# jw007123/hp-Adaptive-Signed-Distance-Field-Octree

Hardware: AMD Instinct MI355X
Metric: Query() Mpts/sec at targetError=1e-5 (union3 field, 10M SplitMix64 pts per GPU, HBM-resident); Create() ms reported as create_ms (higher is better)
Workload: dtype f64

## Files before the change

### hp-adaptive-signed-distance-field-octree_amd/csrc/field_eval.hpp

```cpp
#pragma once
#include <hip/hip_runtime.h>

#include "device_types.hpp"

namespace hpsdf {

template <bool LEFT>
__device__ __forceinline__ double sum3(double a, double b, double c) {
    if constexpr (LEFT) return (a + b) + c;
    else return a + (b + c);
}
template <bool LEFT>
__device__ __forceinline__ double prod3(double a, double b, double c) {
    if constexpr (LEFT) return (a * b) * c;
    else return a * (b * c);
}
__device__ __forceinline__ double sqrtExact(double x) {
    const uint32_t hi = (uint32_t)__double2hiint(x);
    const bool plain = hi - 0x10000000u < 0x7FF00000u - 0x10000000u;
    if (__builtin_amdgcn_ballot_w64(!plain) != 0ull) return sqrt(x);
    const double y = __builtin_amdgcn_rsq(x);
    double g = x * y, h = y * 0.5;
    const double r = __builtin_fma(-h, g, 0.5);
    g = __builtin_fma(g, r, g);
    h = __builtin_fma(h, r, h);
    double d = __builtin_fma(-g, g, x);
    g = __builtin_fma(d, h, g);
    d = __builtin_fma(-g, g, x);
    return __builtin_fma(d, h, g);
}

template <bool LEFT>
__device__ __forceinline__ double norm3(double x, double y, double z) { return sqrtExact(sum3<LEFT>(x * x, y * y, z * z)); }

template <bool LEFT>
__device__ __forceinline__ double primEval(const hpsdf_prim& pr, double x, double y, double z) {
    const double* p = pr.p;
    switch (pr.kind) {
        case HPSDF_PRIM_SPHERE:
            return norm3<LEFT>(x - p[0], y - p[1], z - p[2]) - p[3];
        case HPSDF_PRIM_BOX: {
            const double qx = fabs(x - p[0]) - p[3];
            const double qy = fabs(y - p[1]) - p[4];
            const double qz = fabs(z - p[2]) - p[5];
            const double outside = norm3<LEFT>(fmax(qx, 0.0), fmax(qy, 0.0), fmax(qz, 0.0));
            const double inside = fmin(fmax(qx, fmax(qy, qz)), 0.0);
            return outside + inside;
        }
        case HPSDF_PRIM_TORUS_Y: {
            const double dx = x - p[0], dy = y - p[1], dz = z - p[2];
            const double l = sqrtExact(dx * dx + dz * dz) - p[3];
            return sqrtExact(l * l + dy * dy) - p[4];
        }
        case HPSDF_PRIM_PLANE:
            return (p[0] * x + (p[1] * y + p[2] * z)) + p[3];
        default:
            return 0.0;
    }
}

template <bool LEFT>
__device__ __forceinline__ double analyticEval(const FieldDev& f, double x, double y, double z) {
    double acc = primEval<LEFT>(f.prims[0], x, y, z);
    for (int i = 1; i < f.nPrims; ++i) {
        const double d = primEval<LEFT>(f.prims[i], x, y, z);
        switch (f.prims[i].op) {
            case HPSDF_OP_UNION: acc = fmin(acc, d); break;
            case HPSDF_OP_INTERSECT: acc = fmax(acc, d); break;
            default: acc = fmax(acc, -d); break;
        }
    }
    return acc;
}

}
```

### hp-adaptive-signed-distance-field-octree_amd/csrc/fit_analytic.hip

```cpp
#include "fit_kernels.hpp"

namespace hpsdf {

HPSDF_FIT_KIND_UNIT(, kFieldAnalytic)

}
```

### hp-adaptive-signed-distance-field-octree_amd/csrc/fit_kernels.hpp

```cpp
#pragma once
#include <hip/hip_runtime.h>

#include <cstdint>

#include "device_types.hpp"
#include "field_glue.hpp"
#include "launch.hpp"

namespace hpsdf {


constexpr int kFitPiece = 8;
#ifndef HPSDF_FIT_MIN_WAVES
#define HPSDF_FIT_MIN_WAVES 4
#endif

__device__ __forceinline__ double fitRowAny(double acc, double a1, const double* __restrict__ tk, double n2,
                                            const double* __restrict__ F, int nq) {
    int k = 0;
    for (; k + 4 <= nq; k += 4) {
        const double f0 = F[k], f1 = F[k + 1], f2 = F[k + 2], f3 = F[k + 3];
        const double t0 = tk[k], t1 = tk[k + 1], t2 = tk[k + 2], t3 = tk[k + 3];
        acc = acc + (a1 * t0 * n2) * f0;
        acc = acc + (a1 * t1 * n2) * f1;
        acc = acc + (a1 * t2 * n2) * f2;
        acc = acc + (a1 * t3 * n2) * f3;
    }
    for (; k < nq; ++k) acc = acc + (a1 * tk[k] * n2) * F[k];
    return acc;
}

template <int KIND, bool CSG, int DEG, int R, bool LEFT>
__device__ __forceinline__ void fitBlockBody(const FitBlock blk, const FitTask* __restrict__ tasks, double* __restrict__ arena,
                                             double* __restrict__ errs, double* __restrict__ mirror,
                                             const DeviceTables* __restrict__ T, const FieldDev& field, const RootMap& rm, double* lds) {
    static_assert(R == 1 || DEG > 0, "cell blocking needs a compile-time degree");
    __shared__ double sNl[13 * 11];
    __shared__ double sRec[26];
    __shared__ int32_t sMeshStack[kFitThreads / 64][kMeshStack];
    __shared__ unsigned char sPosI[KIND == kFieldMesh ? 64 : 4], sPosJK[KIND == kFieldMesh ? 64 : 4];
    const int tid = threadIdx.x;
    const int deg = DEG > 0 ? DEG : (int)blk.degree;
    const int nq = 4 * deg + 1, nq2 = nq * nq, G = blk.nTasks;
    const int rowStart = blk.rowStart, rowEnd = blk.rowEnd, nrows = rowEnd - rowStart;
    const int gl = nq * (nq - 1) / 2;
    const int planes = blk.planesPerChunk;
    const int depth = blk.depth;
    const bool split = blk.split != 0;

    double* sT = lds;
    double* sR = sT + (deg + 1) * nq;
    double* sW = sR + nq;
    double* sC = sW + nq;
    double* sF = sC + 8 * G;

    stageQueryTables(T, sNl, sRec);
    for (int q = tid; q < nq; q += kFitThreads) {
        const double x = T->roots[gl + q];
        sR[q] = x;
        sW[q] = T->weights[gl + q];
        double m2 = 0.0, m1 = 1.0;
        sT[q] = 1.0;
        for (int i = 1; i <= deg; ++i) {
            const double l = T->rec[i][0] * x * m1 - T->rec[i][1] * m2;
            m2 = m1, m1 = l;
            sT[i * nq + q] = l;
        }
    }
    for (int g = tid; g < G; g += kFitThreads) {
        const FitTask& tk = tasks[blk.firstTask + g];
        double sc[3];
        for (int a = 0; a < 3; ++a) {
            sc[a] = (double)(tk.bmax[a] - tk.bmin[a]) * 0.5;
            sC[8 * g + 3 + a] = (double)((tk.bmin[a] + tk.bmax[a]) / 2.0f);
            sC[8 * g + a] = sc[a];
        }
        sC[8 * g + 6] = prod3<LEFT>(sc[0], sc[1], sc[2]);
        sC[8 * g + 7] = __longlong_as_double((long long)tk.sampleOff);
    }
    __syncthreads();

    const bool wide = DEG == 0 && nrows > kFitThreads;
    const int slot = wide ? 0 : tid / nrows;
    const int g2 = slot * R;
    const int r0 = rowStart + (wide ? tid : tid % nrows);
    const int r1 = r0 + kFitThreads;
    const bool act0 = wide ? (r0 < rowEnd) : (tid < ((G + R - 1) / R) * nrows);
    const bool act1 = wide && r1 < rowEnd;
    int i0a = 0, i1a = 0, i2a = 0, i0b = 0, i1b = 0, i2b = 0;
    double n0a = 0, n1a = 0, n2a = 0, n0b = 0, n1b = 0, n2b = 0;
    if (act0) {
        i0a = T->bidx[r0][0], i1a = T->bidx[r0][1], i2a = T->bidx[r0][2];
        n0a = sNl[i0a * 11 + depth], n1a = sNl[i1a * 11 + depth], n2a = sNl[i2a * 11 + depth];
    }
    if (act1) {
        i0b = T->bidx[r1][0], i1b = T->bidx[r1][1], i2b = T->bidx[r1][2];
        n0b = sNl[i0b * 11 + depth], n1b = sNl[i1b * 11 + depth], n2b = sNl[i2b * 11 + depth];
    }
    constexpr int NQF = DEG > 0 ? 4 * DEG + 1 : 1;
    double tkReg[NQF];
    if (DEG > 0) {
#pragma unroll
        for (int k = 0; k < NQF; ++k) tkReg[k] = sT[i2a * nq + k];
    }
    uint32_t meshHint = 0xFFFFFFFFu;
    double acc[R];
#pragma unroll
    for (int r = 0; r < R; ++r) acc[r] = 0.0;
    double acc1 = 0.0;

    const int cellStride = planes * nq2;
    for (int iBase = 0; iBase < nq; iBase += planes) {
        const int np = min(planes, nq - iBase);
        if constexpr (KIND == kFieldMesh) {
            if (tid < nq) {
                int rank = 0;
                for (int b = 0; b < nq; ++b) rank += sR[b] < sR[tid] ? 1 : 0;
                sPosJK[rank] = (unsigned char)tid;
            }
            if (tid >= 64 && tid < 64 + np) {
                const int a = tid - 64;
                int rank = 0;
                for (int b = 0; b < np; ++b) rank += sR[iBase + b] < sR[iBase + a] ? 1 : 0;
                sPosI[rank] = (unsigned char)a;
            }
            __syncthreads();
        }
        if constexpr (KIND != kFieldMesh) {
            const int cols = G * nq2;
            for (int c0 = 0; c0 < cols; c0 += kFitThreads) {
                const int cc = c0 + tid;
                const bool activeS = cc < cols;
                const int ccl = activeS ? cc : cols - 1;
                const int g = ccl / nq2, jk = ccl - g * nq2, j = jk / nq, k = jk - j * nq;
                const double* c = sC + 8 * g;
                const double uy = sR[j] * c[1] + c[4], uz = sR[k] * c[2] + c[5];
                const double wy = uy * rm.bounds[1] + rm.centre[1];
                const double wz = uz * rm.bounds[2] + rm.centre[2];
                const double wj = sW[j], wk = sW[k], c6 = c[6];
                const uint64_t sbase = (uint64_t)__double_as_longlong(c[7]) + (uint64_t)(j * nq + k);
                for (int il = 0; il < np; ++il) {
                    const int i = iBase + il;
                    const double ux = sR[i] * c[0] + c[3];
                    const double wx = ux * rm.bounds[0] + rm.centre[0];
                    const uint64_t sidx = sbase + (uint64_t)(i * nq2);
                    const double fv = activeS ? fieldEvalWorld<KIND, CSG, LEFT>(field, wx, wy, wz, sidx, sNl, sRec, meshHint) : 0.0;
                    if (activeS) {
                        sF[g * cellStride + il * nq2 + jk] = c6 * prod3<LEFT>(sW[i], wj, wk) * fv;
                        if (split) const_cast<double*>(field.samples)[sidx] = fv;
                    }
                }
            }
        } else {
            const int chunkSamples = np * nq2, total = G * chunkSamples;
            const float invChunk = 1.0f / (float)chunkSamples;
            for (int s0 = 0; s0 < total; s0 += kFitThreads) {
                const int s = s0 + tid;
                const bool activeS = s < total;
                const int sc = activeS ? s : total - 1;
                int g = (int)(((float)sc + 0.5f) * invChunk);
                int rem = sc - g * chunkSamples;
                if (rem < 0) {
                    --g;
                    rem += chunkSamples;
                } else if (rem >= chunkSamples) {
                    ++g;
                    rem -= chunkSamples;
                }
                if constexpr (KIND == kFieldMesh) rem = meshSampleOrder(rem, np, nq, sPosI, sPosJK);
                const double* c = sC + 8 * g;
                const int il = rem / nq2, jk = rem - il * nq2, j = jk / nq, k = jk - j * nq, i = iBase + il;
                const double ux = sR[i] * c[0] + c[3], uy = sR[j] * c[1] + c[4], uz = sR[k] * c[2] + c[5];
                const double wx = ux * rm.bounds[0] + rm.centre[0];
                const double wy = uy * rm.bounds[1] + rm.centre[1];
                const double wz = uz * rm.bounds[2] + rm.centre[2];
                const uint64_t sidx = (uint64_t)__double_as_longlong(c[7]) + (uint64_t)((i * nq + j) * nq + k);
                double fv;
                if constexpr (KIND == kFieldMesh) {
                    const double mv = (double)meshSignedDistanceWave(field.mesh, V3{(float)wx, (float)wy, (float)wz}, activeS, meshHint,
                                                                     sMeshStack[tid >> 6]);
                    fv = activeS ? applyCsg<CSG>(field, mv, wx, wy, wz, sNl, sRec) : 0.0;
                } else {
                    fv = activeS ? fieldEvalWorld<KIND, CSG, LEFT>(field, wx, wy, wz, sidx, sNl, sRec, meshHint) : 0.0;
                }
                if (activeS) {
                    sF[g * cellStride + rem] = c[6] * prod3<LEFT>(sW[i], sW[j], sW[k]) * fv;
                    if constexpr (KIND != kFieldMesh)
                        if (split) const_cast<double*>(field.samples)[sidx] = fv;
                }
            }
        }
        __syncthreads();
        if (act0) {
            const double* tj = sT + i1a * nq;
            const double* tk = sT + i2a * nq;
            for (int il = 0; il < np; ++il) {
                const double* F = sF + g2 * cellStride + il * nq2;
                const double a0 = sT[i0a * nq + iBase + il] * n0a;
#ifdef HPSDF_FIT_ROW_UNROLL
#pragma unroll HPSDF_FIT_ROW_UNROLL
#endif
                for (int j = 0; j < nq; ++j) {
                    const double a1 = a0 * tj[j] * n1a;
                    if constexpr (DEG > 0 && DEG <= 5) {
                        double lp[NQF];
#pragma unroll
                        for (int k = 0; k < NQF; ++k) lp[k] = a1 * tkReg[k] * n2a;
#pragma unroll
                        for (int r = 0; r < R; ++r) {
                            const double* Fr = F + r * cellStride + j * nq;
                            double f[NQF];
#pragma unroll
                            for (int k = 0; k < NQF; ++k) f[k] = Fr[k];
#pragma unroll
                            for (int k = 0; k < NQF; ++k) acc[r] = acc[r] + lp[k] * f[k];
                        }
                    } else if constexpr (DEG > 5) {
                        const double* Fr = F + j * nq;
#pragma unroll
                        for (int k0 = 0; k0 < NQF; k0 += kFitPiece) {
                            double lp[kFitPiece], f[kFitPiece];
#pragma unroll
                            for (int k = 0; k < kFitPiece; ++k)
                                if (k0 + k < NQF) f[k] = Fr[k0 + k];
#pragma unroll
                            for (int k = 0; k < kFitPiece; ++k)
                                if (k0 + k < NQF) lp[k] = a1 * tkReg[k0 + k] * n2a;
#pragma unroll
                            for (int k = 0; k < kFitPiece; ++k)
                                if (k0 + k < NQF) acc[0] = acc[0] + lp[k] * f[k];
                        }
                    } else {
                        acc[0] = fitRowAny(acc[0], a1, tk, n2a, F + j * nq, nq);
                    }
                }
            }
        }
        if (act1) {
            const double* tj = sT + i1b * nq;
            const double* tk = sT + i2b * nq;
            for (int il = 0; il < np; ++il) {
                const double* F = sF + il * nq2;
                const double a0 = sT[i0b * nq + iBase + il] * n0b;
                for (int j = 0; j < nq; ++j) {
                    const double a1 = a0 * tj[j] * n1b;
                    acc1 = fitRowAny(acc1, a1, tk, n2b, F + j * nq, nq);
                }
            }
        }
        __syncthreads();
    }

    const bool weighted = blk.weighted != 0;
    const int stashStride = weighted ? rowEnd : nrows, stashBase = weighted ? 0 : rowStart;
    const int outBase = split ? 0 : stashBase;
    if (act0) {
#pragma unroll
        for (int r = 0; r < R; ++r)
            if (g2 + r < G) {
                const uint64_t at = tasks[blk.firstTask + g2 + r].outOff + (r0 - outBase);
                arena[at] = acc[r];
                if (mirror != nullptr) mirror[at] = acc[r];
                sF[(g2 + r) * stashStride + (r0 - stashBase)] = acc[r];
            }
    }
    if (act1) {
        arena[tasks[blk.firstTask].outOff + (r1 - outBase)] = acc1;
        sF[r1 - stashBase] = acc1;
    }
    if (weighted && rowStart > 0) {
        for (int s = tid; s < G * rowStart; s += kFitThreads) {
            const int g = s / rowStart, r = s - g * rowStart;
            const FitTask& tk = tasks[blk.firstTask + g];
            const double v = arena[tk.copyOff + r];
            arena[tk.outOff + r] = v;
            sF[g * stashStride + r] = v;
        }
    }
    __syncthreads();
    for (int g = tid; g < G; g += kFitThreads) {
        const int first = deg > 0 ? (int)T->count[deg - 1] : 0;
        double e = 0.0;
        for (int r = first > rowStart ? first : rowStart; r < rowEnd; ++r)
            if (T->bidx[r][3] == deg) {
                const double c = sF[g * stashStride + (r - stashBase)];
                e = e + c * c;
            }
        errs[tasks[blk.firstTask + g].errSlot] = e;
    }
}

template <int KIND, bool CSG, bool LEFT>
__global__ __launch_bounds__(kFitThreads, HPSDF_FIT_MIN_WAVES) void fit_multi_kernel(const FitBlock* __restrict__ blocks,
                                                                const FitTask* __restrict__ tasks, double* __restrict__ arena,
                                                                double* __restrict__ errs, const DeviceTables* __restrict__ T,
                                                                FieldDev field, RootMap rm, const uint32_t* __restrict__ count,
                                                                uint32_t countValue) {
    extern __shared__ double lds[];
    const uint32_t n = count ? *count : countValue;
    if (blockIdx.x >= n) return;
    const FitBlock blk = blocks[n - 1u - blockIdx.x];
    switch (blk.degree) {
        case 2: fitBlockBody<KIND, CSG, 2, 1, LEFT>(blk, tasks, arena, errs, nullptr, T, field, rm, lds); break;
        case 3: fitBlockBody<KIND, CSG, 3, 1, LEFT>(blk, tasks, arena, errs, nullptr, T, field, rm, lds); break;
        case 4: fitBlockBody<KIND, CSG, 4, 1, LEFT>(blk, tasks, arena, errs, nullptr, T, field, rm, lds); break;
        case 5: fitBlockBody<KIND, CSG, 5, 1, LEFT>(blk, tasks, arena, errs, nullptr, T, field, rm, lds); break;
        case 6: fitBlockBody<KIND, CSG, 6, 1, LEFT>(blk, tasks, arena, errs, nullptr, T, field, rm, lds); break;
        case 7: fitBlockBody<KIND, CSG, 7, 1, LEFT>(blk, tasks, arena, errs, nullptr, T, field, rm, lds); break;
        case 8: fitBlockBody<KIND, CSG, 8, 1, LEFT>(blk, tasks, arena, errs, nullptr, T, field, rm, lds); break;
        default: fitBlockBody<KIND, CSG, 0, 1, LEFT>(blk, tasks, arena, errs, nullptr, T, field, rm, lds); break;
    }
}

template <int KIND, bool CSG, int DEG, int R, bool LEFT>
__global__ __launch_bounds__(kFitThreads, HPSDF_FIT_MIN_WAVES) void fit_kernel(const FitBlock* __restrict__ blocks,
                                                          const FitTask* __restrict__ tasks, double* __restrict__ arena,
                                                          double* __restrict__ errs, double* __restrict__ mirror,
                                                          const DeviceTables* __restrict__ T, FieldDev field, RootMap rm,
                                                          const uint32_t* __restrict__ range) {
    extern __shared__ double lds[];
    uint32_t b = blockIdx.x;
    if (range != nullptr) {
        if (b >= range[1]) return;
        b += range[0];
    }
    fitBlockBody<KIND, CSG, DEG, R, LEFT>(blocks[b], tasks, arena, errs, mirror, T, field, rm, lds);
}

template <int KIND, bool CSG, bool LEFT>
__global__ __launch_bounds__(256) void field_kernel(FieldDev f, const DeviceTables* __restrict__ T,
                                                    const double* __restrict__ xyz, size_t n, double* __restrict__ out) {
    __shared__ double sNl[13 * 11];
    __shared__ double sRec[26];
    stageQueryTables(T, sNl, sRec);
    __syncthreads();
    const size_t stride = (size_t)gridDim.x * blockDim.x;
    uint32_t hint = 0xFFFFFFFFu;
    for (size_t i = (size_t)blockIdx.x * blockDim.x + threadIdx.x; i < n; i += stride)
        out[i] = fieldEvalWorld<KIND, CSG, LEFT>(f, xyz[3 * i], xyz[3 * i + 1], xyz[3 * i + 2], i, sNl, sRec, hint);
}

template <int KIND, bool CSG, bool LEFT>
// ... 83 lines not shown
```

### hp-adaptive-signed-distance-field-octree_amd/csrc/frontier.hip

```cpp
#include <hip/hip_runtime.h>

#include <algorithm>
#include <atomic>
#include <cfloat>
#include <cmath>
#include <cstddef>
#include <chrono>
#include <cstdio>
#include <cstdlib>
#include <cstring>
#include <memory>
#include <vector>

#include "block.hpp"
#include "builder.hpp"
#include "frontier.hpp"
#include "launch.hpp"
#include "runtime.hpp"

namespace hpsdf {

namespace {

constexpr uint32_t kFrJobs = 4096;
// ... 98 lines not shown
    int32_t fastFit;
    int32_t splitFit;
    uint64_t sampleCap;
    uint32_t buildStamp;
    uint32_t stamps;
    double target;
    int32_t weighted;
    int32_t replica;
    double* means;
    const double* weights;
    uint32_t* hostFlag;
};

__host__ __device__ inline uint32_t frCoef(int p) { return p == 6 ? 83u : (uint32_t)((p + 1) * (p + 2) * (p + 3) / 6); }
__host__ __device__ inline int frClass(int degree, bool incr, int depth) { return (2 * degree + (incr ? 1 : 0)) * kFrDepths + depth; }
__host__ __device__ inline size_t frLds(int degree, int g, int planes) {
    const size_t nq = 4 * (size_t)degree + 1;
    return ((size_t)(degree + 1) * nq + 2 * nq + 8 * (size_t)g + (size_t)g * planes * nq * nq) * sizeof(double);
}
constexpr size_t kFrFitLdsCap = 45 * 1024;
__host__ __device__ inline bool frSplit(int splitFit, int degree, bool incr) { return splitFit > 0 && !incr && degree >= splitFit && degree <= 11; }
__host__ __device__ inline void frShape(int degree, bool incr, uint32_t count, int* cells, int* planes, bool fast = false, bool weighted = false,
                                        int split = 0) {
    if (fast && degree >= 4 && degree <= 11) {
        *cells = kMfmaCells, *planes = 1;
        return;
    }
    if (frSplit(split, degree, incr)) incr = true;
    const int nrows = incr ? (int)(frCoef(degree) - frCoef(degree - 1)) : (int)frCoef(degree);
    int gmax = nrows > kFitBlockThreads ? 1 : kFitBlockThreads / nrows;
    while (gmax > 1 && frLds(degree, gmax, 1) > (weighted ? kFitMaxLdsBytes : kFrFitLdsCap)) --gmax;
    uint32_t spread = (count + 511u) / 512u;
    int cap = gmax;
    if (degree == 2) {
        if (count <= 4096u) spread = (count + 1023u) / 1024u;
        cap = gmax < 16 ? gmax : 16;
    }
    int g = (int)(spread < 1u ? 1u : spread);
    g = g < cap ? g : cap;
    const int nq = 4 * degree + 1;
    int pl = nq;
    while (pl > 1 && frLds(degree, g, pl) > kFitChunkLdsBytes) --pl;
    if (weighted) {
        const int need = (int)frCoef(degree) + 100;
        const int minPlanes = (need + nq * nq - 1) / (nq * nq);
        const int want = nq < minPlanes ? nq : minPlanes;
        pl = pl > want ? pl : want;
        while (g > 1 && frLds(degree, g, pl) > kFitMaxLdsBytes) --g;
    }
    *cells = g;
    *planes = pl;
}

__device__ __forceinline__ size_t frErrSlot(const FrDev& d, const FrHdr* h, uint32_t j) {
    if (d.world == 1) return (size_t)j * 9;
    const uint32_t o = d.jobOwner[j];
    return (size_t)o * d.errStride + (size_t)(j - h->sliceFirst[o]) * 9;
}
__device__ __forceinline__ double* frStatusSlot(const FrDev& d, int r) { return d.errs + (size_t)r * d.errStride + (d.errStride - 1u); }
__device__ __forceinline__ void frPeerCheck(const FrDev& d, uint32_t* sPeer) {
    if (d.world > 1 && threadIdx.x < (uint32_t)d.world &&
        (unsigned long long)__double_as_longlong(*(volatile double*)frStatusSlot(d, (int)threadIdx.x)) == ~0ull)
        atomicMax(sPeer, threadIdx.x + 1u);
}
__device__ __forceinline__ uint64_t frJobCost(int degree, int depth, bool coarse) {
    auto cube = [](uint64_t n) { return n * n * n; };
    if (coarse) return frCoef(2) * cube(9);
    uint64_t c = 0;
    if (depth < kMaxDepth) c += 8ull * frCoef(degree) * cube(4 * (uint64_t)degree + 1);
    if (degree < kMaxDegree - 1) c += (uint64_t)(frCoef(degree + 1) - frCoef(degree)) * cube(4 * (uint64_t)degree + 5);
    return c ? c : 1;
}

__device__ __forceinline__ uint32_t frDigit(int level, uint64_t bits, uint32_t idx) {
    switch (level) {
        case 0: return (uint32_t)(bits >> 52) & 2047u;
        case 1: return (uint32_t)(bits >> 41) & 2047u;
        case 2: return (uint32_t)(bits >> 30) & 2047u;
        case 3: return (uint32_t)(bits >> 19) & 2047u;
        case 4: return (uint32_t)(bits >> 8) & 2047u;
        case 5: return (uint32_t)bits & 255u;
        case 6: return (~idx >> 21) & 2047u;
        case 7: return (~idx >> 10) & 2047u;
        default: return ~idx & 1023u;
    }
}

__device__ void frThreshold(const uint32_t* hist, uint32_t need, uint32_t* , int* outT, uint32_t* outAbove) {
    if (threadIdx.x < 64) {
        const int lane = (int)threadIdx.x;
        uint32_t own = 0;
        for (int k = 0; k < 32; ++k) own += hist[lane * 32 + k];
        uint32_t suf = own;
        for (int off = 1; off < 64; off <<= 1) {
            const uint32_t v = __shfl_down(suf, off, 64);
            if (lane + off < 64) suf += v;
        }
        const uint32_t aboveLane = suf - own;
        const bool crossing = aboveLane < need && need <= suf;
        const unsigned long long m = __ballot(crossing);
        if (m == 0ull) {
            if (lane == 0) *outT = -1, *outAbove = suf;
        } else if (crossing) {
            uint32_t cum = aboveLane;
            int bb = lane * 32 + 31;
            for (; bb > lane * 32 && cum + hist[bb] < need; --bb) cum += hist[bb];
// ... 1435 lines not shown
        d.segFirst[i] = 2;
    }
    if (blockIdx.x != 0) return;
    if (threadIdx.x == 0 && d.world > 1) *frStatusSlot(d, d.rank) = 0.0;
    uint32_t* hw = reinterpret_cast<uint32_t*>(d.hdr);
    for (uint32_t w = threadIdx.x; w < sizeof(FrHdr) / 4; w += 256u) hw[w] = 0;
    __syncthreads();
    if (threadIdx.x == 0) {
        FrHdr* h = d.hdr;
        h->nNodes = t.nNodes;
        h->nJobs = t.nLeaves;
        h->nLeaves = t.nLeaves;
        h->t1 = -1;
        h->total = 4096.0 * HPSDF_INITIAL_NODE_ERR;
        h->maxDegree = 2;
        h->nTasks = t.nTasks, h->nBlocks = t.nBlocks;
        h->degTasks[2][0] = 0, h->degTasks[2][1] = t.nTasks;
        h->degBlocks[2][0] = 0, h->degBlocks[2][1] = t.nBlocks;
        h->arenaUsed = t.arenaRows;
        h->sampleUsed = t.samples;
        h->fits = t.nTasks, h->samples = t.samples;
        h->nCoeffs = (uint64_t)t.nLeaves * frCoef(2);
        for (int r = 0; r < 9; ++r) h->sliceFirst[r] = t.sliceFirst[r];
    }
    if (d.world > 1)
        for (uint32_t j = threadIdx.x; j < t.nLeaves; j += 256u) {
            uint32_t o = 0;
            for (int r = 1; r < d.world; ++r) o += t.sliceFirst[r] <= j ? 1u : 0u;
            d.jobOwner[j] = (uint8_t)o;
        }
}

}

struct FrontierWorkspace {
    int device = -1;
    bool inUse = false;
    FrDev d{};
    FrHdr* hostHdr = nullptr;
    uint32_t nodeCap = 0;
    uint64_t arenaCap = 0, sampleCap = 0;
    double* arena = nullptr;
    double* samples = nullptr;
    FrTemplate tmpl{};
    hpsdf_node* tmplNodes = nullptr;
    uint32_t* tmplParent = nullptr;
    uint32_t* tmplSub = nullptr;
    uint32_t* tmplLeaves = nullptr;
    double* tmplErr = nullptr;
    uint64_t* tmplJobP = nullptr;
    FitTask* tmplTasks = nullptr;
    FitBlock* tmplBlocks = nullptr;
    size_t tmplLds = 0;
    bool clean = false;
    bool lastWentOn = false;
    int cleanRank = -1, cleanWorld = -1;
    uint32_t buildStamp = 0;
    std::vector<hpsdf_node> hostNodesAfterRound0;
    char* pinned = nullptr;
    double* pinnedDev = nullptr;
    size_t pinnedCap = 0;
    double* hostMeans = nullptr;
    double* hostWeights = nullptr;
    uint32_t* hostFlag = nullptr;
    uint32_t flagStamp = 0;
    hipError_t ensureWeighting() {
        if (hostMeans) return hipSuccess;
        const size_t n = 8 * ((size_t)kFrJobs * HPSDF_JOB_HEADER_DOUBLES + kFrStatusPad);
        hipError_t e = hipHostMalloc((void**)&hostMeans, n * sizeof(double), hipHostMallocCoherent | hipHostMallocMapped);
        if (e == hipSuccess) e = hipHostMalloc((void**)&hostWeights, n * sizeof(double), hipHostMallocCoherent | hipHostMallocMapped);
        if (e == hipSuccess) e = hipHostMalloc((void**)&hostFlag, 64, hipHostMallocCoherent | hipHostMallocMapped);
        if (e == hipSuccess) e = hipHostGetDevicePointer((void**)&d.means, hostMeans, 0);
        if (e == hipSuccess) e = hipHostGetDevicePointer((void**)&d.weights, hostWeights, 0);
        if (e == hipSuccess) e = hipHostGetDevicePointer((void**)&d.hostFlag, hostFlag, 0);
        if (e == hipSuccess) {
            std::memset(hostMeans, 0, n * sizeof(double));
            for (size_t i = 0; i < n; ++i) hostWeights[i] = 1.0;
            hostFlag[0] = hostFlag[1] = 0;
        }
        return e;
    }
    static constexpr int kSide = 3;
    hipStream_t side[kSide] = {nullptr, nullptr, nullptr};
    hipEvent_t forkEv = nullptr, joinEv[kSide] = {nullptr, nullptr, nullptr};

    template <typename T>
    static hipError_t grow(T** p, size_t oldCount, size_t newCount, hipStream_t s, bool keep) {
        T* np = nullptr;
        hipError_t e = hipMalloc((void**)&np, newCount * sizeof(T));
        if (e != hipSuccess) return e;
        if (*p) {
            if (keep && oldCount) e = hipMemcpyAsync(np, *p, oldCount * sizeof(T), hipMemcpyDeviceToDevice, s);
            if (e == hipSuccess) e = hipStreamSynchronize(s);
            (void)hipFree(*p);
        }
        *p = np;
        return e;
    }
    static constexpr uint64_t kBytesPerNode = sizeof(hpsdf_node) + sizeof(uint64_t)  + 2 * sizeof(uint32_t)  +
                                              (uint64_t)kFrSegs * sizeof(uint64_t)  + sizeof(uint64_t)  + 2 * sizeof(uint32_t) ;
    hipError_t ensureNodes(uint32_t need, hipStream_t s) {
        if (need <= nodeCap) return hipSuccess;
        uint32_t nc = nodeCap ? nodeCap : 65536u;
        while (nc < need) nc *= 2;
        hipError_t e = grow(&d.nodes, nodeCap, nc, s, true);
        if (e == hipSuccess) e = grow(&d.qErr, nodeCap, nc, s, true);
// ... 66 lines not shown
        size_t nc = pinnedCap ? pinnedCap : (1u << 20);
        while (nc < need) nc *= 2;
        if (pinned) (void)hipHostFree(pinned);
        pinned = nullptr, pinnedDev = nullptr, pinnedCap = 0;
        hipError_t e = hipHostMalloc((void**)&pinned, nc, hipHostMallocCoherent | hipHostMallocMapped);
        if (e == hipSuccess) e = hipHostGetDevicePointer((void**)&pinnedDev, pinned, 0);
        if (e == hipSuccess) pinnedCap = nc;
        return e;
    }
    template <typename T>
    static hipError_t upload(T** dst, const std::vector<T>& v) {
        hipError_t e = hipMalloc((void**)dst, std::max<size_t>(1, v.size()) * sizeof(T));
        if (e == hipSuccess && !v.empty()) e = hipMemcpy(*dst, v.data(), v.size() * sizeof(T), hipMemcpyHostToDevice);
        return e;
    }
    hipError_t init(int dev, hipStream_t s) {
        device = dev;
        hipError_t e = hipMalloc((void**)&d.hdr, sizeof(FrHdr));
        if (e == hipSuccess) e = hipMalloc((void**)&d.rnd, sizeof(FrRound));
        if (e == hipSuccess) e = hipHostMalloc((void**)&hostHdr, sizeof(FrHdr), hipHostMallocCoherent | hipHostMallocMapped);
        if (e == hipSuccess) e = hipHostGetDevicePointer((void**)&d.hostHdr, hostHdr, 0);
        if (e == hipSuccess) e = hipMalloc((void**)&d.taken, (kFrJobs + 64) * sizeof(uint32_t));
        if (e == hipSuccess) e = hipMalloc((void**)&d.wBatchIdx, kFrJobs * sizeof(uint32_t));
        if (e == hipSuccess) e = hipMalloc((void**)&d.wBatchErr, kFrJobs * sizeof(double));
        if (e == hipSuccess) e = hipMalloc((void**)&d.wJobP, kFrJobs * sizeof(uint64_t));
        if (e == hipSuccess) e = hipMalloc((void**)&d.wJobH, kFrJobs * sizeof(uint64_t));
        if (e == hipSuccess) e = hipMalloc((void**)&d.ops, (size_t)kFrJobs * 9 * sizeof(double));
        if (e == hipSuccess) e = hipMalloc((void**)&d.jobRecA, kFrJobs * sizeof(uint32_t));
        if (e == hipSuccess) e = hipMalloc((void**)&d.jobRecB, kFrJobs * sizeof(uint16_t));
        if (e == hipSuccess) e = hipMalloc((void**)&d.tasks, kFrTasks * sizeof(FitTask));
        if (e == hipSuccess) e = hipMalloc((void**)&d.blocks, kFrTasks * sizeof(FitBlock));
        if (e == hipSuccess) e = hipMalloc((void**)&d.errs, (size_t)kFrJobs * HPSDF_JOB_HEADER_DOUBLES * sizeof(double));
        if (e != hipSuccess) return e;
        d.batchIdx = d.wBatchIdx, d.batchErr = d.wBatchErr, d.jobP = d.wJobP, d.jobH = d.wJobH;
        hpsdf_build b;
        hpsdf_config cfg;
        hpsdf_config_default(&cfg);
        cfg.thread_count = 1;
        if (builderBegin(&b, &cfg, nullptr) != HPSDF_OK) return hipErrorUnknown;
        const uint32_t nT = (uint32_t)b.nodes.size();
        std::vector<uint32_t> parent(nT, 0), leaves, sub(nT, 0);
        for (uint32_t i = 0; i < nT; ++i) {
            if (b.nodes[i].child_idx != ~0ull)
                for (unsigned c = 0; c < 8; ++c) parent[b.nodes[i].child_idx + c] = i;
            else
                leaves.push_back(i);
        }
        const uint32_t nL = (uint32_t)leaves.size();
        if (nL > kFrJobs) return hipErrorUnknown;
        for (uint32_t i = nT; i-- > 1;) {
            const uint32_t own = b.nodes[i].child_idx == ~0ull ? frCoef(2) : sub[i];
            sub[parent[i]] += own;
        }
        int g = 1, pl = 1;
        frShape(2, false, nL, &g, &pl);
        std::vector<FitTask> tasks(nL);
        std::vector<uint64_t> jobP(nL);
        std::vector<double> errs(nL, HPSDF_INITIAL_NODE_ERR);
        for (uint32_t j = 0; j < nL; ++j) {
            const hpsdf_node& n = b.nodes[leaves[j]];
            FitTask& t = tasks[j];
            std::memset(&t, 0, sizeof t);
            for (int a = 0; a < 3; ++a) t.bmin[a] = n.aabb_min[a], t.bmax[a] = n.aabb_max[a];
            t.outOff = (uint64_t)j * frCoef(2);
            t.copyOff = ~0ull;
            t.sampleOff = (uint64_t)j * 729;
            t.errSlot = j * HPSDF_JOB_HEADER_DOUBLES;
            t.depth = n.depth;
            t.pad[0] = 2;
            jobP[j] = t.outOff;
        }
        std::vector<FitBlock> blocks((nL + g - 1) / g);
        for (uint32_t k = 0; k < blocks.size(); ++k) {
            FitBlock& fb = blocks[k];
            std::memset(&fb, 0, sizeof fb);
            fb.firstTask = k * (uint32_t)g;
            fb.nTasks = (uint16_t)std::min<uint32_t>((uint32_t)g, nL - k * (uint32_t)g);
            fb.degree = 2;
            fb.planesPerChunk = (uint8_t)pl;
            fb.rowStart = 0, fb.rowEnd = (uint16_t)frCoef(2);
            fb.depth = b.nodes[leaves[0]].depth;
        }
        tmplLds = frLds(2, g, pl);
        hostTmplTasks = tasks;
        hostNodesAfterRound0 = b.nodes;
        for (uint32_t j = 0; j < nL; ++j) {
            hostNodesAfterRound0[leaves[j]].degree = 2;
            hostNodesAfterRound0[leaves[j]].coeffs_start = (uint64_t)j * frCoef(2);
        }
        e = upload(&tmplNodes, b.nodes);
        if (e == hipSuccess) e = upload(&tmplParent, parent);
        if (e == hipSuccess) e = upload(&tmplSub, sub);
        if (e == hipSuccess) e = upload(&tmplLeaves, leaves);
        if (e == hipSuccess) e = upload(&tmplErr, errs);
        if (e == hipSuccess) e = upload(&tmplJobP, jobP);
        if (e == hipSuccess) e = upload(&tmplTasks, tasks);
        if (e == hipSuccess) e = upload(&tmplBlocks, blocks);
        tmpl.nodes = tmplNodes, tmpl.parent = tmplParent, tmpl.sub = tmplSub;
        tmpl.nNodes = nT, tmpl.nLeaves = nL, tmpl.nTasks = nL, tmpl.nBlocks = (uint32_t)blocks.size();
        tmpl.arenaRows = (uint64_t)nL * frCoef(2), tmpl.samples = (uint64_t)nL * 729;
        for (int k = 0; k < kSide && e == hipSuccess; ++k) {
            e = hipStreamCreateWithFlags(&side[k], hipStreamNonBlocking);
            if (e == hipSuccess) e = hipEventCreateWithFlags(&joinEv[k], hipEventDisableTiming);
        }
        if (e == hipSuccess) e = hipEventCreateWithFlags(&forkEv, hipEventDisableTiming);
        if (e == hipSuccess) e = ensureNodes(65536, s);
        if (e == hipSuccess) e = ensureArena(1ull << 22, 0, s);
        if (e == hipSuccess) e = ensurePinned(4u << 20);
// ... 200 lines not shown
            std::atomic_thread_fence(std::memory_order_acquire);
            if (flag[1] != stamp) return fail(HPSDF_ERR_STATE, "frontier: the round's means did not arrive");
        }
        const double tw = now();
        tSync += tw - ts;
        const uint32_t nJobs = world == 1 ? std::min<uint32_t>(ws->hostFlag[0], kFrJobs) : std::min<uint32_t>(nMine, kFrJobs);
        const double dd = std::sqrt(3.0), strength = cfg.weighting_strength;
        const double* mean = ws->hostMeans + base;
        double* w = ws->hostWeights + base;
        const uint32_t step = round0 ? 9u : 1u;
        for (uint32_t i = 0; i < nJobs * 9u; i += step) {
            if (cfg.weighting_type == 1) {
                const double k = std::pow(1.0 - mean[i] / dd, strength);
                w[i] = std::min<double>(1.0, std::max<double>(k, 0.0));
            } else {
                w[i] = std::exp(-1.0 * strength * mean[i] / dd);
            }
        }
        std::atomic_thread_fence(std::memory_order_release);
        tWeights += now() - tw;
        FR_LAUNCH(fr_weigh_kernel, dim3((std::max(1u, nJobs) * 9u + 255u) / 256u), dim3(256), s, d, round0 ? 1u : 9u, base, nJobs * 9u);
        return HPSDF_OK;
    };
    uint8_t* early = nullptr;
    bool earlyCopied = false;
    struct FreeEarly {
        hpsdf_ctx* ctx;
        uint8_t** p;
        ~FreeEarly() { ctx->freeBlock(*p); }
    } freeEarly{ctx, &early};
    FrTemplate T0 = T;
    const FitTask* r0Tasks = ws->tmplTasks;
    const FitBlock* r0Blocks = ws->tmplBlocks;
    const uint64_t* r0JobP = ws->tmplJobP;
    size_t r0Lds = ws->tmplLds;
    uint64_t part0 = 0;
    T0.sliceFirst[0] = 0;
    for (int r = 1; r < 9; ++r) T0.sliceFirst[r] = T.nLeaves;
    if (world > 1) {
        const uint64_t c = (uint64_t)frCoef(2) * 729ull, total = c * T.nLeaves;
        uint32_t start = 0;
        for (int r = 0; r < world; ++r) {
            uint32_t end = T.nLeaves;
            if (r + 1 < world) {
                const uint64_t target = total * (uint64_t)(r + 1) / (uint64_t)world;
                end = (uint32_t)((target + c - 1) / c);
                end = std::min(std::max(end, start), T.nLeaves);
            }
            T0.sliceFirst[r + 1] = end;
            start = end;
        }
        const uint32_t first = T0.sliceFirst[rank], count = T0.sliceFirst[rank + 1] - first;
        int g = 1, pl = 1;
        frShape(2, false, std::max(1u, count), &g, &pl);
        const uint32_t nBl = (count + (uint32_t)g - 1u) / (uint32_t)g;
        uint32_t maxCount = 1;
        for (int r = 0; r < world; ++r) maxCount = std::max(maxCount, T0.sliceFirst[r + 1] - T0.sliceFirst[r]);
        part0 = ((uint64_t)maxCount * frCoef(2) + 15ull) & ~15ull;
        if (ws->r0Rank != rank || ws->r0World != world || ws->r0ErrStride != ws->d.errStride || ws->r0Replica != replica) {
            std::vector<FitTask>& tk = ws->hostR0Tasks;
            tk.assign(ws->hostTmplTasks.begin() + first, ws->hostTmplTasks.begin() + first + count);
            std::vector<uint64_t> jobP(T.nLeaves, ~0ull & kOffMask);
            for (uint32_t q = 0; q < count; ++q) {
                tk[q].outOff = (replica ? (uint64_t)rank * part0 : 0ull) + (uint64_t)q * frCoef(2);
                tk[q].sampleOff = (uint64_t)q * 729;
                tk[q].errSlot = (uint32_t)rank * ws->d.errStride + q * HPSDF_JOB_HEADER_DOUBLES;
                jobP[first + q] = tk[q].outOff;
            }
            if (replica)
                for (int r = 0; r < world; ++r)
                    for (uint32_t j = T0.sliceFirst[r]; j < T0.sliceFirst[r + 1]; ++j) jobP[j] = (uint64_t)r * part0 + (uint64_t)(j - T0.sliceFirst[r]) * frCoef(2);
            std::vector<FitBlock> bl(nBl);
            for (uint32_t k = 0; k < bl.size(); ++k) {
                FitBlock& fb = bl[k];
                std::memset(&fb, 0, sizeof fb);
                fb.firstTask = k * (uint32_t)g;
                fb.nTasks = (uint16_t)std::min<uint32_t>((uint32_t)g, count - k * (uint32_t)g);
                fb.degree = 2;
                fb.planesPerChunk = (uint8_t)pl;
                fb.rowStart = 0, fb.rowEnd = (uint16_t)frCoef(2);
                fb.depth = ws->hostTmplTasks[0].depth;
            }
            ws->r0Rank = ws->r0World = -1;
            HPSDF_HIP(hipMemcpyAsync(ws->r0Tasks, tk.data(), count * sizeof(FitTask), hipMemcpyHostToDevice, s));
            HPSDF_HIP(hipMemcpyAsync(ws->r0Blocks, bl.data(), bl.size() * sizeof(FitBlock), hipMemcpyHostToDevice, s));
            HPSDF_HIP(hipMemcpyAsync(ws->r0JobP, jobP.data(), jobP.size() * sizeof(uint64_t), hipMemcpyHostToDevice, s));
            HPSDF_HIP(hipStreamSynchronize(s));
            ws->r0Rank = rank, ws->r0World = world, ws->r0ErrStride = ws->d.errStride, ws->r0Replica = replica;
        }
        r0Tasks = ws->r0Tasks, r0Blocks = ws->r0Blocks, r0JobP = ws->r0JobP;
        r0Lds = frLds(2, g, pl);
        T0.nTasks = count, T0.nBlocks = nBl;
        T0.arenaRows = replica ? (uint64_t)world * part0 : (uint64_t)count * frCoef(2), T0.samples = (uint64_t)count * 729;
    }
    const uint32_t stride0 = kFrJobs * HPSDF_JOB_HEADER_DOUBLES + kFrStatusPad, strideK = Kj * HPSDF_JOB_HEADER_DOUBLES + kFrStatusPad;
    const uint32_t inlineNodes = [] {
        const char* e = std::getenv("HPSDF_FRONTIER_INLINE_NODES");
        return e ? (uint32_t)std::strtoul(e, nullptr, 10) : kFrInlineNodes;
    }();
    bool splitOpen = false, samplesTooLarge = false;
    uint64_t measuredLimit = 0;
    auto prepareNext = [&](uint32_t knownNodes, uint64_t knownArena, uint32_t knownMaxDeg, int roundsDone) -> int {
        const int degBound = (int)std::min<uint32_t>(knownMaxDeg + 1u, kMaxDegree);
        const uint64_t needNodes = (uint64_t)knownNodes + 8ull * Kj;
        const uint64_t needArena = knownArena + (replica ? (uint64_t)world * ((uint64_t)Kj * rowsPerJob(degBound) + 16) : (uint64_t)Kj * rowsPerJob(degBound));
        {
            const uint64_t needSamples = mesh ? std::min<uint64_t>((uint64_t)Kj * samplesPerJob(degBound), 1ull << 31) : 0ull;
// ... 341 lines not shown
```

Before: 94580.

## Evaluate analytic field over plane segments per thread in degree-2 fit blocks

For the analytic, non-CSG degree-2 fit path, each thread now evaluates the field at up to three x-planes for one (j,k) column. The primitive switch is hoisted outside the per-point loop so the per-primitive branch and y/z setup are amortised. The error reduction uses a precomputed bitmask of top-degree rows instead of looping over table rows. It also adds an env-var override for the round-0 block shape and optional timestamp instrumentation, which is compiled out by default. These changes only touch Create(); Query throughput should be unaffected, apart from register pressure risk in the fit kernel.

```diff
diff --git a/hp-adaptive-signed-distance-field-octree_amd/csrc/field_eval.hpp b/hp-adaptive-signed-distance-field-octree_amd/csrc/field_eval.hpp
--- a/hp-adaptive-signed-distance-field-octree_amd/csrc/field_eval.hpp
+++ b/hp-adaptive-signed-distance-field-octree_amd/csrc/field_eval.hpp
@@ -73,4 +73,48 @@
     return acc;
 }
 
+template <bool LEFT, int N>
+__device__ __forceinline__ void primEvalPlanes(const hpsdf_prim& pr, const double (&x)[N], int n, double y, double z, double (&d)[N]) {
+#define HPSDF_PRIM_PLANES               \
+    _Pragma("unroll") for (int q = 0; q < N; ++q) \
+        if (q < n) d[q] = primEval<LEFT>(pr, x[q], y, z)
+    switch (pr.kind) {
+        case HPSDF_PRIM_SPHERE: HPSDF_PRIM_PLANES; break;
+        case HPSDF_PRIM_BOX: HPSDF_PRIM_PLANES; break;
+        case HPSDF_PRIM_TORUS_Y: HPSDF_PRIM_PLANES; break;
+        case HPSDF_PRIM_PLANE: HPSDF_PRIM_PLANES; break;
+        default: HPSDF_PRIM_PLANES; break;
+    }
+#undef HPSDF_PRIM_PLANES
 }
+template <bool LEFT, int N>
+__device__ __forceinline__ void analyticEvalPlanes(const FieldDev& f, const double (&x)[N], int n, double y, double z, double (&acc)[N]) {
+    static_assert(N >= 1 && N <= 3, "a handful of points: each keeps its coordinates and two values in registers");
+#pragma unroll
+    for (int q = 0; q < N; ++q) acc[q] = 0.0;
+    const hpsdf_prim first = f.prims[0];
+    primEvalPlanes<LEFT, N>(first, x, n, y, z, acc);
+    for (int i = 1; i < f.nPrims; ++i) {
+        const hpsdf_prim pr = f.prims[i];
+        double d[N];
+#pragma unroll
+        for (int q = 0; q < N; ++q) d[q] = 0.0;
+        primEvalPlanes<LEFT, N>(pr, x, n, y, z, d);
+        switch (pr.op) {
+            case HPSDF_OP_UNION:
+#pragma unroll
+                for (int q = 0; q < N; ++q) acc[q] = fmin(acc[q], d[q]);
+                break;
+            case HPSDF_OP_INTERSECT:
+#pragma unroll
+                for (int q = 0; q < N; ++q) acc[q] = fmax(acc[q], d[q]);
+                break;
+            default:
+#pragma unroll
+                for (int q = 0; q < N; ++q) acc[q] = fmax(acc[q], -d[q]);
+                break;
+        }
+    }
+}
+
+}
diff --git a/hp-adaptive-signed-distance-field-octree_amd/csrc/fit_analytic.hip b/hp-adaptive-signed-distance-field-octree_amd/csrc/fit_analytic.hip
--- a/hp-adaptive-signed-distance-field-octree_amd/csrc/fit_analytic.hip
+++ b/hp-adaptive-signed-distance-field-octree_amd/csrc/fit_analytic.hip
@@ -5,3 +5,17 @@
 HPSDF_FIT_KIND_UNIT(, kFieldAnalytic)
 
 }
+
+#ifdef HPSDF_FIT_STAMPS_BUILD
+extern "C" __attribute__((visibility("default"))) int hpsdf_lab_fit_stamps(unsigned long long* out, size_t count, int clear) {
+    const size_t all = sizeof hpsdf::gFitStamps / sizeof hpsdf::gFitStamps[0];
+    if (count > all) return 1;
+    if (hipDeviceSynchronize() != hipSuccess) return 3;
+    if (out && hipMemcpyFromSymbol(out, HIP_SYMBOL(hpsdf::gFitStamps), count * sizeof *out) != hipSuccess) return 3;
+    if (clear) {
+        void* p = nullptr;
+        if (hipGetSymbolAddress(&p, HIP_SYMBOL(hpsdf::gFitStamps)) != hipSuccess || hipMemset(p, 0, sizeof hpsdf::gFitStamps) != hipSuccess) return 3;
+    }
+    return 0;
+}
+#endif
diff --git a/hp-adaptive-signed-distance-field-octree_amd/csrc/fit_kernels.hpp b/hp-adaptive-signed-distance-field-octree_amd/csrc/fit_kernels.hpp
--- a/hp-adaptive-signed-distance-field-octree_amd/csrc/fit_kernels.hpp
+++ b/hp-adaptive-signed-distance-field-octree_amd/csrc/fit_kernels.hpp
@@ -11,8 +11,23 @@
 
 
 constexpr int kFitPiece = 8;
+constexpr int kFitSegment = 3;
 #ifndef HPSDF_FIT_MIN_WAVES
 #define HPSDF_FIT_MIN_WAVES 4
+#endif
+
+#ifdef HPSDF_FIT_STAMPS_BUILD
+constexpr int kFitStampSlots = 16, kFitStampGroups = 4096, kFitStampDepth = 4, kFitStampPasses = 6;
+__device__ unsigned long long gFitStamps[kFitStampGroups * (kFitThreads / 64) * kFitStampSlots];
+__device__ __forceinline__ void fitStampValue(bool on, int slot, unsigned long long v) {
+    if (on && (threadIdx.x & 63) == 0 && blockIdx.x < (unsigned)kFitStampGroups)
+        gFitStamps[(blockIdx.x * (kFitThreads / 64) + (threadIdx.x >> 6)) * kFitStampSlots + slot] = v;
+}
+#define HPSDF_FIT_STAMP(on, slot) fitStampValue(on, slot, __builtin_amdgcn_s_memtime())
+#define HPSDF_FIT_STAMP_VALUE(on, slot, v) fitStampValue(on, slot, (unsigned long long)(v))
+#else
+#define HPSDF_FIT_STAMP(on, slot) ((void)0)
+#define HPSDF_FIT_STAMP_VALUE(on, slot, v) ((void)0)
 #endif
 
 __device__ __forceinline__ double fitRowAny(double acc, double a1, const double* __restrict__ tk, double n2,
@@ -47,6 +62,10 @@
     const int planes = blk.planesPerChunk;
     const int depth = blk.depth;
     const bool split = blk.split != 0;
+#ifdef HPSDF_FIT_STAMPS_BUILD
+    const bool stamped = depth == kFitStampDepth;
+#endif
+    HPSDF_FIT_STAMP(stamped, 0);
 
     double* sT = lds;
     double* sR = sT + (deg + 1) * nq;
@@ -79,6 +98,7 @@
         sC[8 * g + 7] = __longlong_as_double((long long)tk.sampleOff);
     }
     __syncthreads();
+    HPSDF_FIT_STAMP(stamped, 1);
 
     const bool wide = DEG == 0 && nrows > kFitThreads;
     const int slot = wide ? 0 : tid / nrows;
@@ -109,6 +129,21 @@
     for (int r = 0; r < R; ++r) acc[r] = 0.0;
     double acc1 = 0.0;
 
+    constexpr bool kCoarse = KIND == kFieldAnalytic && !CSG && DEG == 2 && R == 1;
+    constexpr int kTopRows = (DEG + 1) * (DEG + 2) / 2;
+    int errFirst = 0;
+    uint32_t topMask = 0;
+    if constexpr (kCoarse) {
+        errFirst = max((int)T->count[DEG - 1], rowStart);
+        if (tid < G) {
+            unsigned char top[kTopRows];
+#pragma unroll
+            for (int q = 0; q < kTopRows; ++q) top[q] = T->bidx[min(errFirst + q, rowEnd - 1)][3];
+#pragma unroll
+            for (int q = 0; q < kTopRows; ++q) topMask |= ((errFirst + q < rowEnd ? 1u : 0u) & (top[q] == deg ? 1u : 0u)) << q;
+        }
+    }
+
     const int cellStride = planes * nq2;
     for (int iBase = 0; iBase < nq; iBase += planes) {
         const int np = min(planes, nq - iBase);
@@ -126,7 +161,42 @@
             }
             __syncthreads();
         }
-        if constexpr (KIND != kFieldMesh) {
+        if constexpr (kCoarse) {
+            const int cols = G * nq2, segs = (np + kFitSegment - 1) / kFitSegment, units = cols * segs;
+            for (int u0 = 0; u0 < units; u0 += kFitThreads) {
+                const int u = u0 + tid;
+                if (u < units) {
+                    const int sg = (u >= cols ? 1 : 0) + (u >= 2 * cols ? 1 : 0), cc = u - sg * cols;
+                    const int g = cc / nq2, jk = cc - g * nq2, j = jk / nq, k = jk - j * nq;
+                    const double* c = sC + 8 * g;
+                    const double uy = sR[j] * c[1] + c[4], uz = sR[k] * c[2] + c[5];
+                    const double wy = uy * rm.bounds[1] + rm.centre[1];
+                    const double wz = uz * rm.bounds[2] + rm.centre[2];
+                    const double wj = sW[j], wk = sW[k], c6 = c[6];
+                    const uint64_t sbase = (uint64_t)__double_as_longlong(c[7]) + (uint64_t)(j * nq + k);
+                    const int il0 = sg * kFitSegment, n = min(kFitSegment, np - il0);
+                    double wx[kFitSegment], fv[kFitSegment];
+#pragma unroll
+                    for (int q = 0; q < kFitSegment; ++q) {
+                        wx[q] = 0.0;
+                        if (q < n) {
+                            const double ux = sR[iBase + il0 + q] * c[0] + c[3];
+                            wx[q] = ux * rm.bounds[0] + rm.centre[0];
+                        }
+                    }
+                    analyticEvalPlanes<LEFT, kFitSegment>(field, wx, n, wy, wz, fv);
+#pragma unroll
+                    for (int q = 0; q < kFitSegment; ++q)
+                        if (q < n) {
+                            const int il = il0 + q, i = iBase + il;
+                            sF[g * cellStride + il * nq2 + jk] = c6 * prod3<LEFT>(sW[i], wj, wk) * fv[q];
+                            if (split) const_cast<double*>(field.samples)[sbase + (uint64_t)(i * nq2)] = fv[q];
+                        }
+                }
+                HPSDF_FIT_STAMP(stamped && iBase == 0 && u0 / kFitThreads < kFitStampPasses, 2 + u0 / kFitThreads);
+            }
+            HPSDF_FIT_STAMP_VALUE(stamped && iBase == 0, 12, (units + kFitThreads - 1) / kFitThreads);
+        } else if constexpr (KIND != kFieldMesh) {
             const int cols = G * nq2;
             for (int c0 = 0; c0 < cols; c0 += kFitThreads) {
                 const int cc = c0 + tid;
@@ -150,7 +220,9 @@
                         if (split) const_cast<double*>(field.samples)[sidx] = fv;
                     }
                 }
-            }
+                HPSDF_FIT_STAMP(stamped && iBase == 0 && c0 / kFitThreads < kFitStampPasses, 2 + c0 / kFitThreads);
+            }
+            HPSDF_FIT_STAMP_VALUE(stamped && iBase == 0, 12, (cols + kFitThreads - 1) / kFitThreads);
         } else {
             const int chunkSamples = np * nq2, total = G * chunkSamples;
             const float invChunk = 1.0f / (float)chunkSamples;
@@ -191,6 +263,7 @@
             }
         }
         __syncthreads();
+        HPSDF_FIT_STAMP(stamped && iBase == 0, 8);
         if (act0) {
             const double* tj = sT + i1a * nq;
             const double* tk = sT + i2a * nq;
@@ -248,8 +321,10 @@
                 }
             }
         }
+        HPSDF_FIT_STAMP(stamped && iBase == 0, 9);
         __syncthreads();
     }
+    HPSDF_FIT_STAMP(stamped, 10);
 
     const bool weighted = blk.weighted != 0;
     const int stashStride = weighted ? rowEnd : nrows, stashBase = weighted ? 0 : rowStart;
@@ -278,16 +353,30 @@
         }
     }
     __syncthreads();
-    for (int g = tid; g < G; g += kFitThreads) {
-        const int first = deg > 0 ? (int)T->count[deg - 1] : 0;
-        double e = 0.0;
-        for (int r = first > rowStart ? first : rowStart; r < rowEnd; ++r)
-            if (T->bidx[r][3] == deg) {
-                const double c = sF[g * stashStride + (r - stashBase)];
-                e = e + c * c;
-            }
-        errs[tasks[blk.firstTask + g].errSlot] = e;
-    }
+    if constexpr (kCoarse) {
+        if (tid < G) {
+            double e = 0.0;
+#pragma unroll
+            for (int q = 0; q < kTopRows; ++q)
+                if (topMask >> q & 1u) {
+                    const double c = sF[tid * stashStride + (errFirst + q - stashBase)];
+                    e = e + c * c;
+                }
+            errs[tasks[blk.firstTask + tid].errSlot] = e;
+        }
+    } else {
+        for (int g = tid; g < G; g += kFitThreads) {
+            const int first = deg > 0 ? (int)T->count[deg - 1] : 0;
+            double e = 0.0;
+            for (int r = first > rowStart ? first : rowStart; r < rowEnd; ++r)
+                if (T->bidx[r][3] == deg) {
+                    const double c = sF[g * stashStride + (r - stashBase)];
+                    e = e + c * c;
+                }
+            errs[tasks[blk.firstTask + g].errSlot] = e;
+        }
+    }
+    HPSDF_FIT_STAMP(stamped, 11);
 }
 
 template <int KIND, bool CSG, bool LEFT>
diff --git a/hp-adaptive-signed-distance-field-octree_amd/csrc/frontier.hip b/hp-adaptive-signed-distance-field-octree_amd/csrc/frontier.hip
--- a/hp-adaptive-signed-distance-field-octree_amd/csrc/frontier.hip
+++ b/hp-adaptive-signed-distance-field-octree_amd/csrc/frontier.hip
@@ -174,6 +174,15 @@
     *planes = pl;
 }
 
+inline void frRound0Shape(uint32_t count, int forced, int* cells, int* planes) {
+    frShape(2, false, count, cells, planes);
+    if (forced <= 0) return;
+    int g = std::min(forced, kFitBlockThreads / (int)frCoef(2)), pl = 9;
+    while (g > 1 && frLds(2, g, 1) > kFrFitLdsCap) --g;
+    while (pl > 1 && frLds(2, g, pl) > kFitChunkLdsBytes) --pl;
+    *cells = g, *planes = pl;
+}
+
 __device__ __forceinline__ size_t frErrSlot(const FrDev& d, const FrHdr* h, uint32_t j) {
     if (d.world == 1) return (size_t)j * 9;
     const uint32_t o = d.jobOwner[j];
@@ -1715,6 +1724,7 @@
     FitTask* tmplTasks = nullptr;
     FitBlock* tmplBlocks = nullptr;
     size_t tmplLds = 0;
+    int r0Cells = 0;
     bool clean = false;
     bool lastWentOn = false;
     int cleanRank = -1, cleanWorld = -1;
@@ -1887,8 +1897,9 @@
             const uint32_t own = b.nodes[i].child_idx == ~0ull ? frCoef(2) : sub[i];
             sub[parent[i]] += own;
         }
+        if (const char* fg = std::getenv("HPSDF_FIT_G")) r0Cells = std::max(0, std::atoi(fg));
         int g = 1, pl = 1;
-        frShape(2, false, nL, &g, &pl);
+        frRound0Shape(nL, r0Cells, &g, &pl);
         std::vector<FitTask> tasks(nL);
         std::vector<uint64_t> jobP(nL);
         std::vector<double> errs(nL, HPSDF_INITIAL_NODE_ERR);
@@ -2195,7 +2206,7 @@
         }
         const uint32_t first = T0.sliceFirst[rank], count = T0.sliceFirst[rank + 1] - first;
         int g = 1, pl = 1;
-        frShape(2, false, std::max(1u, count), &g, &pl);
+        frRound0Shape(std::max(1u, count), ws->r0Cells, &g, &pl);
         const uint32_t nBl = (count + (uint32_t)g - 1u) / (uint32_t)g;
         uint32_t maxCount = 1;
         for (int r = 0; r < world; ++r) maxCount = std::max(maxCount, T0.sliceFirst[r + 1] - T0.sliceFirst[r]);
```

Result: no change. 95000 (median of 5 runs) (+0.4%).
